# Chriz122/ultralytics_pro

Measured on AMD Instinct MI355X. Metric: images/sec (whole job = n_gpus x per-GPU bs=32) YOLOv8n 640x640 (forward + Detect decode + NMS), higher is better.
Workload: dtype bf16

## Files before the change

### include/upa.h

```cpp
#ifndef UPA_H
#define UPA_H
#include <stddef.h>
#include <stdint.h>

#ifdef __cplusplus
extern "C" {
#endif

enum { UPA_F32 = 0, UPA_BF16 = 1, UPA_U8_BGR_HWC = 2  };
enum { UPA_ACT_NONE = 0, UPA_ACT_SILU = 1, UPA_ACT_RELU = 2 };
enum { UPA_OK = 0, UPA_EINVAL = -1, UPA_EUNSUPPORTED = -2, UPA_EWORKSPACE = -3, UPA_ELAUNCH = -4 };

typedef struct upa_opts {
  uint32_t size;
  int32_t conv_big;
  int32_t conv_big_bm;
  int32_t conv_ckt;
  int32_t no_ws, no_pipe, no_1x1, no_c16, no_upcat;
  int32_t pipe_all;
  int32_t pipe_min_tiles;
  int32_t pipe_wgs, c16_wgs;
  int32_t c1_mt, c1_waves, c1_wgs;
  int32_t pair;
  int32_t pair_tile64, pair_tile32;
  int32_t no_pair_cv2;
  int32_t c2f;
  int32_t c2f16_waves;
  int32_t c2f32_th;
  int32_t no_branch_tail;
  int32_t branch_tail_bm;
  int32_t stem_wgs, stemf_wgs, stemf_waves, stem_no_mfma;
  int32_t ablate_conv, ablate_pipe, ablate_c1, ablate_stem;
  int32_t c2f64_max_px;
  int32_t conv_ws3;
  int32_t no_group;
  int32_t no_c2f32_up;
  int32_t no_xcd;
  int32_t keys_only;
  int32_t conv_p8;
  int32_t c2f_stream;
  int32_t c2f_stream_rows;
  int32_t no_stack_first;
  int32_t no_epi_stats;
  int32_t nms_stages;
  int32_t nms_first_prefix;
  int32_t detect_stream;
  int32_t detect_stream_rows;
  int32_t no_sppf_front;
  int32_t no_c2f16_down;
} upa_opts;

int upa_version(void);
const char* upa_last_error(void);
size_t upa_opts_size(void);

size_t upa_conv_packed_weight_bytes(int cout, int cin, int k, int dtype);
int upa_pack_conv_weight(const float* w_oihw, int cout, int cin, int k, int dtype, void* out);
int upa_conv2d_bias_act(const void* x, int n, int h, int w, int cin, int ldx,
                        const void* w_packed, const float* bias ,
                        void* y, int cout, int ldy,
                        const void* residual , int ldr,
                        int k, int stride, int pad, int act, int dtype, const upa_opts* opts, void* stream);
typedef struct upa_conv_problem {
  const void* x; int32_t n, h, w, cin, ldx;
  const void* w_packed; const float* bias;
  void* y; int32_t cout, ldy;
  const void* residual; int32_t ldr;
} upa_conv_problem;
int upa_conv2d_bias_act_group(const upa_conv_problem* probs, int count, int k, int stride, int pad, int act, int dtype,
                              const upa_opts* opts, void* stream);

int upa_conv2d_pool2(const void* x, int n, int h, int w, int cin, int ldx, const void* w_packed, const float* bias, void* y, int cout,
                     int ldy, int k, int stride, int pad, int act, int dtype, const upa_opts* opts, void* stream);
int upa_conv2d_stem_nchw_pool2(const void* x_nchw, int x_dtype, int n, int cin, int h, int w, const float* w_oihw, const float* bias,
                               void* y, int cout, int ldy, int k, int stride, int pad, int act, int dtype, const upa_opts* opts,
                               void* stream);

int upa_conv_variant(int n, int h, int w, int cin, int cout, int k, int stride, int pad, int dtype, const upa_opts* opts);

int upa_bottleneck_pair(const void* x, int n, int h, int w, int c, int ldx, const void* w1_packed, const float* b1,
                        const void* w2_packed, const float* b2, void* y, int ldy, int residual, int act, int dtype,
                        const upa_opts* opts, void* stream);
int upa_bottleneck_pair_e(const void* x, int n, int h, int w, int c, int cmid, int ldx, const void* w1_packed, const float* b1,
                          const void* w2_packed, const float* b2, void* y, int ldy, int residual, int act, int dtype,
                          const upa_opts* opts, void* stream);


size_t upa_stem_packed_weight_bytes(int cout, int cin, int k);
int upa_pack_stem_weight(const float* w_oihw, int cout, int cin, int k, float* out );
int upa_conv2d_stem_nchw(const void* x_nchw, int x_dtype, int n, int cin, int h, int w,
                         const float* w_oihw, const float* bias, void* y, int cout, int ldy,
                         int k, int stride, int pad, int act, int dtype, const upa_opts* opts, void* stream);

int upa_stem_conv_fused(const void* x, int n, int h, int w, const float* w0, const float* b0, const void* w1,
                        const float* b1, void* y, int ldy, const upa_opts* opts, void* stream);
int upa_stem_conv_fused_k(const void* x, int n, int h, int w, int k0, const float* w0, const float* b0, const void* w1,
                          const float* b1, void* y, int ldy, const upa_opts* opts, void* stream);
int upa_stem_conv_fused_c(const void* x, int n, int h, int w, int k0, int c0, const float* w0, const float* b0, const void* w1,
                          const float* b1, void* y, int ldy, const upa_opts* opts, void* stream);
int upa_stem_conv_fused_s(const void* x, int n, int h, int w, int k0, int s0, int c0, const float* w0, const float* b0,
                          const void* w1, const float* b1, void* y, int ldy, const upa_opts* opts, void* stream);

int upa_maxpool2d(const void* x, int n, int h, int w, int c, int ldx, void* y, int oh, int ow, int ldy,
                  int k, int stride, int pad, int pad_br, int dtype, void* stream);
int upa_sppf_pool3(const void* x, int n, int h, int w, int c, int ldx, void* y1, void* y2, void* y3, int ldy,
                   int dtype, void* stream);
int upa_sppf_front(const void* x, int n, int h, int w, int c1, int ldx, const void* w_packed, const float* bias, void* y, int c_, int ldy, int dtype,
                   const upa_opts* opts, void* stream);
int upa_upsample2x(const void* x, int n, int h, int w, int c, int ldx, void* y, int ldy, int dtype, void* stream);
int upa_copy_view(const void* x, int n, int h, int w, int c, int ldx, void* y, int ldy, int dtype, void* stream);
int upa_copy_to_host(const void* src_dev, void* dst_pinned, size_t bytes, void* stream);
int upa_results_to_host(const void* rows_dev, const int* counts_dev, int batch, int max_rows, int row_bytes,
                        void* rows_pinned, int* counts_pinned, void* stream);
int upa_add_view(const void* a, int lda, const void* b, int ldb, void* y, int ldy, int n, int h, int w, int c,
                 int dtype, void* stream);
int upa_nchw_to_nhwc(const float* x, int n, int c, int h, int w, void* y, int ldy, int dtype, void* stream);
int upa_nhwc_to_nchw(const void* x, int n, int h, int w, int c, int ldx, float* y, int dtype, void* stream);
int upa_letterbox_u8(const void* src, int n, int h0, int w0, long src_image_stride, int src_row_stride, void* dst, int H, int W,
                     int new_h, int new_w, int top, int left, int pad_value, void* stream);


int upa_detect_decode(const void* box, int ldb, const void* cls, int ldc, int n, int h, int w, int reg_max, int nc,
                      float stride_px, float* y, int a_total, int a0, int dtype, void* stream);
int upa_detect_tail(const void* x, int n, int h, int w, int cin, int ldx, const void* w_packed, const float* bias, int cout,
                    int kind, int nc, float stride_px, float* y, int a_total, int a0, void* raw, int ldraw,
                    unsigned long long* best_keys, int dtype, const upa_opts* opts, void* stream);

int upa_conv1x1_upcat(const void* x, int n, int h, int w, int cin, int ldx, const void* up, int up_c, int up_ld,
                      const void* w_packed, const float* bias, void* y, int cout, int ldy, int act, int dtype,
                      const upa_opts* opts, void* stream);

int upa_bottleneck_pair_cv2(const void* x, const void* y0, int n, int h, int w, int ldx, const void* w1_packed, const float* b1,
                            const void* w2_packed, const float* b2, int residual, const void* wc_std, const void* wc_b,
                            const float* bc, void* out, int ldout, int act, int dtype, const upa_opts* opts, void* stream);

int upa_c2f_fused(const void* x, int n, int h, int w, int c1, int ldx, int c, int nb, int shortcut, const void* w1,
                  const float* b1, const void* const* wm, const float* const* bm, const void* w2, const float* b2, void* y,
                  int c2, int ldy, int act, int dtype, const upa_opts* opts, void* stream);

int upa_c2f16_down_fused(const void* x, int n, int h, int w, int ldx, const void* w1, const float* b1, const void* const* wm,
                         const float* const* bm, const void* w2, const float* b2, const void* wd, const float* bd, void* y, int ldy,
                         int dtype, const upa_opts* opts, void* stream);

int upa_c2f64_fused(const void* x, int n, int h, int w, int c1, int ldx, const void* up, int up_c, int up_ld, int nb, int shortcut,
                    const void* w1, const float* b1, const void* const* wm, const float* const* bm, const void* w2,
                    const float* b2, void* y, int c2, int ldy, int act, int dtype, const upa_opts* opts, void* stream);
int upa_c2f32_up_fused(const void* x, int n, int h, int w, int c1, int ldx, const void* up, int up_c, int up_ld, int nb, int shortcut,
                       const void* w1, const float* b1, const void* const* wm, const float* const* bm, const void* w2, const float* b2,
                       void* y, int c2, int ldy, int act, int dtype, const upa_opts* opts, void* stream);

size_t upa_tail_packed_weight_bytes(int cout, int cin);
int upa_pack_tail_weight(const float* w, int cout, int cin, void* out);
int upa_detect_branch_tail(const void* x, int n, int h, int w, int c, int ldx, const void* w3_packed, const float* b3,
                           const void* wt_packed, const float* bt, int kind, int nc, float stride_px, float* y, int a_total,
                           int a0, unsigned long long* best_keys, int dtype, const upa_opts* opts, void* stream);
typedef struct upa_branch_level {
  const void* x; int32_t n, h, w, c, ldx;
  const void* w3_packed; const float* b3;
  const void* wt_packed; const float* bt;
  float stride_px; int32_t a0;
} upa_branch_level;
// ... 168 lines not shown
```

### ultralytics_pro_amd/_lib.py

```python

from __future__ import annotations

import ctypes as C
import os
from pathlib import Path

import torch

UPA_F32, UPA_BF16, UPA_U8_BGR_HWC = 0, 1, 2
UPA_EUNSUPPORTED = -2
ACT_NONE, ACT_SILU, ACT_RELU = 0, 1, 2

_PKG = Path(__file__).resolve().parent
LIB_PATH = Path(os.environ.get("UPA_HIP_LIB", _PKG / "libupa_hip.so"))

_vp, _i, _f, _sz = C.c_void_p, C.c_int, C.c_float, C.c_size_t


class Opts(C.Structure):

    _fields_ = [("size", C.c_uint32), ("conv_big", _i), ("conv_big_bm", _i), ("conv_ckt", _i),
                ("no_ws", _i), ("no_pipe", _i), ("no_1x1", _i), ("no_c16", _i), ("no_upcat", _i),
                ("pipe_all", _i), ("pipe_min_tiles", _i), ("pipe_wgs", _i), ("c16_wgs", _i),
                ("c1_mt", _i), ("c1_waves", _i), ("c1_wgs", _i),
                ("pair", _i), ("pair_tile64", _i), ("pair_tile32", _i), ("no_pair_cv2", _i),
                ("c2f", _i), ("c2f16_waves", _i), ("c2f32_th", _i),
                ("no_branch_tail", _i), ("branch_tail_bm", _i),
                ("stem_wgs", _i), ("stemf_wgs", _i), ("stemf_waves", _i), ("stem_no_mfma", _i),
                ("ablate_conv", _i), ("ablate_pipe", _i), ("ablate_c1", _i), ("ablate_stem", _i), ("c2f64_max_px", _i), ("conv_ws3", _i), ("no_group", _i), ("no_c2f32_up", _i), ("no_xcd", _i), ("keys_only", _i), ("conv_p8", _i), ("c2f_stream", _i), ("c2f_stream_rows", _i), ("no_stack_first", _i), ("no_epi_stats", _i), ("nms_stages", _i), ("nms_first_prefix", _i), ("detect_stream", _i), ("detect_stream_rows", _i), ("no_sppf_front", _i), ("no_c2f16_down", _i)]

    def __init__(self, **kw):
        super().__init__()
        self.size = C.sizeof(Opts)
        for k, v in kw.items():
            if k in dict(self._fields_):
                setattr(self, k, int(v))
            else:
                raise AttributeError(f"upa_opts has no field '{k}'")

    def replace(self, **kw) -> "Opts":
        o = Opts()
        C.memmove(C.byref(o), C.byref(self), C.sizeof(Opts))
        for k, v in kw.items():
            setattr(o, k, int(v))
        return o

    _ENV = {"UPA_CONV_BIG": ("conv_big", lambda v: {0: 1, 1: 0, 2: 2}[int(v)]), "UPA_CONV_BIG_BM": ("conv_big_bm", int), "UPA_CONV_WS3": ("conv_ws3", int),
            "UPA_CONV_CKT": ("conv_ckt", int), "UPA_CONV_NO_WS": ("no_ws", lambda v: 1), "UPA_CONV_NO_PIPE": ("no_pipe", lambda v: 1),
            "UPA_CONV_NO_1X1": ("no_1x1", lambda v: 1), "UPA_CONV_NO_C16": ("no_c16", lambda v: 1), "UPA_NO_UPCAT": ("no_upcat", lambda v: 1),
            "UPA_PIPE_ALL": ("pipe_all", lambda v: 1), "UPA_PIPE_MIN_TILES": ("pipe_min_tiles", int), "UPA_PIPE_WGS": ("pipe_wgs", int),
            "UPA_C16_WGS": ("c16_wgs", int), "UPA_C1_MT": ("c1_mt", int), "UPA_C1_WAVES": ("c1_waves", int), "UPA_C1_WGS": ("c1_wgs", int),
            "UPA_NO_PAIR": ("pair", lambda v: {0: 2, 1: 1, 2: 0, 3: 3}[int(v)]), "UPA_PAIR_T64": ("pair_tile64", int),
            "UPA_PAIR_T32": ("pair_tile32", int), "UPA_NO_PAIR_CV2": ("no_pair_cv2", int), "UPA_NO_C2F": ("c2f", int),
            "UPA_C2F16_WAVES": ("c2f16_waves", int), "UPA_C2F32_TH": ("c2f32_th", int), "UPA_NO_BRANCH_TAIL": ("no_branch_tail", int),
            "UPA_BRANCH_TAIL_BM": ("branch_tail_bm", int), "UPA_STEM_WGS": ("stem_wgs", int), "UPA_STEMF_WGS": ("stemf_wgs", int),
            "UPA_STEMF_WAVES": ("stemf_waves", int), "UPA_STEM_NO_MFMA": ("stem_no_mfma", lambda v: 1),
            "UPA_CONV_ABLATE": ("ablate_conv", int), "UPA_PIPE_ABLATE": ("ablate_pipe", int), "UPA_C1_ABLATE": ("ablate_c1", int),
            "UPA_STEM_ABLATE": ("ablate_stem", int)}

    @classmethod
    def from_env(cls, env=None) -> "Opts":
        env = os.environ if env is None else env
        o = cls()
        for name, (field, conv) in cls._ENV.items():
            if name in env:
                setattr(o, field, conv(env[name]))
        return o


class BranchLevel(C.Structure):
    _fields_ = [("x", C.c_void_p), ("n", _i), ("h", _i), ("w", _i), ("c", _i), ("ldx", _i), ("w3_packed", C.c_void_p), ("b3", C.c_void_p),
                ("wt_packed", C.c_void_p), ("bt", C.c_void_p), ("stride_px", C.c_float), ("a0", _i)]


class DetectBranch(C.Structure):
    _fields_ = [("c", _i), ("reserved", _i), ("w1", C.c_void_p), ("b1", C.c_void_p), ("w2", C.c_void_p), ("b2", C.c_void_p),
                ("wt", C.c_void_p), ("bt", C.c_void_p)]


class ConvProblem(C.Structure):
    _fields_ = [("x", C.c_void_p), ("n", _i), ("h", _i), ("w", _i), ("cin", _i), ("ldx", _i), ("w_packed", C.c_void_p), ("bias", C.c_void_p),
                ("y", C.c_void_p), ("cout", _i), ("ldy", _i), ("residual", C.c_void_p), ("ldr", _i)]


_op = C.POINTER(Opts)

PROTOTYPES = {
    "upa_version": (_i, []),
    "upa_last_error": (C.c_char_p, []),
    "upa_opts_size": (_sz, []),
    "upa_conv_packed_weight_bytes": (_sz, [_i, _i, _i, _i]),
    "upa_pack_conv_weight": (_i, [_vp, _i, _i, _i, _i, _vp]),
    "upa_conv2d_bias_act": (_i, [_vp, _i, _i, _i, _i, _i, _vp, _vp, _vp, _i, _i, _vp, _i, _i, _i, _i, _i, _i, _op, _vp]),
    "upa_conv_variant": (_i, [_i, _i, _i, _i, _i, _i, _i, _i, _i, _op]),
    "upa_bottleneck_pair": (_i, [_vp, _i, _i, _i, _i, _i, _vp, _vp, _vp, _vp, _vp, _i, _i, _i, _i, _op, _vp]),
    "upa_bottleneck_pair_e": (_i, [_vp, _i, _i, _i, _i, _i, _i, _vp, _vp, _vp, _vp, _vp, _i, _i, _i, _i, _op, _vp]),
    "upa_stem_packed_weight_bytes": (_sz, [_i, _i, _i]),
    "upa_pack_stem_weight": (_i, [_vp, _i, _i, _i, _vp]),
    "upa_conv2d_stem_nchw": (_i, [_vp, _i, _i, _i, _i, _i, _vp, _vp, _vp, _i, _i, _i, _i, _i, _i, _i, _op, _vp]),
    "upa_conv2d_stem_nchw_pool2": (_i, [_vp, _i, _i, _i, _i, _i, _vp, _vp, _vp, _i, _i, _i, _i, _i, _i, _i, _op, _vp]),
    "upa_conv2d_pool2": (_i, [_vp, _i, _i, _i, _i, _i, _vp, _vp, _vp, _i, _i, _i, _i, _i, _i, _i, _op, _vp]),
    "upa_stem_conv_fused": (_i, [_vp, _i, _i, _i, _vp, _vp, _vp, _vp, _vp, _i, _op, _vp]),
    "upa_stem_conv_fused_k": (_i, [_vp, _i, _i, _i, _i, _vp, _vp, _vp, _vp, _vp, _i, _op, _vp]),
    "upa_stem_conv_fused_c": (_i, [_vp, _i, _i, _i, _i, _i, _vp, _vp, _vp, _vp, _vp, _i, _op, _vp]),
    "upa_stem_conv_fused_s": (_i, [_vp, _i, _i, _i, _i, _i, _i, _vp, _vp, _vp, _vp, _vp, _i, _op, _vp]),
    "upa_maxpool2d": (_i, [_vp, _i, _i, _i, _i, _i, _vp, _i, _i, _i, _i, _i, _i, _i, _i, _vp]),
    "upa_sppf_pool3": (_i, [_vp, _i, _i, _i, _i, _i, _vp, _vp, _vp, _i, _i, _vp]),
    "upa_upsample2x": (_i, [_vp, _i, _i, _i, _i, _i, _vp, _i, _i, _vp]),
    "upa_copy_view": (_i, [_vp, _i, _i, _i, _i, _i, _vp, _i, _i, _vp]),
    "upa_copy_to_host": (_i, [_vp, _vp, _sz, _vp]),
    "upa_results_to_host": (_i, [_vp, _vp, _i, _i, _i, _vp, _vp, _vp]),
    "upa_add_view": (_i, [_vp, _i, _vp, _i, _vp, _i, _i, _i, _i, _i, _i, _vp]),
    "upa_nchw_to_nhwc": (_i, [_vp, _i, _i, _i, _i, _vp, _i, _i, _vp]),
    "upa_nhwc_to_nchw": (_i, [_vp, _i, _i, _i, _i, _i, _vp, _i, _vp]),
    "upa_letterbox_u8": (_i, [_vp, _i, _i, _i, C.c_long, _i, _vp, _i, _i, _i, _i, _i, _i, _i, _vp]),
    "upa_detect_decode": (_i, [_vp, _i, _vp, _i, _i, _i, _i, _i, _i, _f, _vp, _i, _i, _i, _vp]),
    "upa_detect_branch_tail_group": (_i, [_vp, _i, _i, _i, _vp, _i, _vp, _i, _op, _vp]),
    "upa_detect_head_tails": (_i, [_vp, _vp, _i, _i, _vp, _i, _vp, _i, _op, _vp]),
    "upa_conv2d_bias_act_group": (_i, [_vp, _i, _i, _i, _i, _i, _i, _op, _vp]),
    "upa_detect_level_stream": (_i, [_vp, _i, _i, _i, _i, _i, _vp, _vp, _i, _f, _vp, _i, _i, _vp, _i, _op, _vp]),
    "upa_detect_tail": (_i, [_vp, _i, _i, _i, _i, _i, _vp, _vp, _i, _i, _i, _f, _vp, _i, _i, _vp, _i, _vp, _i, _op, _vp]),
    "upa_conv1x1_upcat": (_i, [_vp, _i, _i, _i, _i, _i, _vp, _i, _i, _vp, _vp, _vp, _i, _i, _i, _i, _op, _vp]),
    "upa_bottleneck_pair_cv2": (_i, [_vp, _vp, _i, _i, _i, _i, _vp, _vp, _vp, _vp, _i, _vp, _vp, _vp, _vp, _i, _i, _i, _op, _vp]),
    "upa_sppf_front": (_i, [_vp, _i, _i, _i, _i, _i, _vp, _vp, _vp, _i, _i, _i, _op, _vp]),
    "upa_c2f16_down_fused": (_i, [_vp, _i, _i, _i, _i, _vp, _vp, _vp, _vp, _vp, _vp, _vp, _vp, _vp, _i, _i, _op, _vp]),
    "upa_c2f_fused": (_i, [_vp, _i, _i, _i, _i, _i, _i, _i, _i, _vp, _vp, _vp, _vp, _vp, _vp, _vp, _i, _i, _i, _i, _op, _vp]),
    "upa_c2f64_fused": (_i, [_vp, _i, _i, _i, _i, _i, _vp, _i, _i, _i, _i, _vp, _vp, _vp, _vp, _vp, _vp, _vp, _i, _i, _i, _i, _op, _vp]),
    "upa_c2f32_up_fused": (_i, [_vp, _i, _i, _i, _i, _i, _vp, _i, _i, _i, _i, _vp, _vp, _vp, _vp, _vp, _vp, _vp, _i, _i, _i, _i, _op, _vp]),
    "upa_tail_packed_weight_bytes": (_sz, [_i, _i]),
    "upa_pack_tail_weight": (_i, [_vp, _i, _i, _vp]),
    "upa_detect_branch_tail": (_i, [_vp, _i, _i, _i, _i, _i, _vp, _vp, _vp, _vp, _i, _i, _f, _vp, _i, _i, _vp, _i, _op, _vp]),
    "upa_nms_batched_hot": (_i, [_vp, _i, _i, _i, _f, _f, _i, _i, _vp, _i, _i, _f, _vp, _vp, _vp, _vp, _sz, _vp, _vp]),
    "upa_nms_workspace_bytes": (_sz, [_i, _i, _i, _i, _i]),
    "upa_nms_batched": (_i, [_vp, _i, _i, _i, _f, _f, _i, _i, _vp, _i, _i, _f, _vp, _vp, _vp, _vp, _sz, _vp]),
    "upa_nms_batched_opts": (_i, [_vp, _i, _i, _i, _f, _f, _i, _i, _vp, _i, _i, _f, _vp, _vp, _vp, _vp, _sz, _vp, _vp]),
    "upa_mhsa": (_i, [_vp, _vp, _vp, _i, _i, _i, _i, _i, _f, _vp, _i, _vp, _i, _i, _vp]),
    "upa_dwconv2d": (_i, [_vp, _i, _i, _i, _i, _i, _vp, _vp, _vp, _i, _i, _i, _i, _i, _i, _vp]),
    "upa_psa_attention": (_i, [_vp, _i, _i, _i, _i, _i, _i, _i, _f, _vp, _vp, _vp, _i, _i, _vp]),
    "upa_linear": (_i, [_vp, C.c_long, _i, _i, _vp, _vp, _vp, _i, _i, _vp, _i, _i, _vp]),
    "upa_linear_bf16": (_i, [_vp, C.c_long, _i, _i, _vp, _vp, _vp, _i, _i, _vp, _i, _i, _vp]),
    "upa_linear_mixed": (_i, [_vp, _i, C.c_long, _i, _i, _vp, _vp, _vp, _i, _i, _i, _vp, _i, _i, _vp]),
    "upa_layer_norm": (_i, [_vp, _vp, _i, _i, _vp, _vp, _f, _vp, _vp]),
    "upa_rows_add": (_i, [_vp, _vp, _vp, C.c_long, _i, _vp]),
    "upa_rows_scale": (_i, [_vp, _vp, _vp, C.c_long, _i, _vp]),
    "upa_rows_gather": (_i, [_vp, _vp, _vp, C.c_long, _i, _vp]),
    "upa_topk_tokens": (_i, [_vp, _i, _i, _vp, _i, _i, _vp, _vp, _vp]),
    "upa_box_refine": (_i, [_vp, _vp, _vp, C.c_long, _vp]),
    "upa_box_add_anchors": (_i, [_vp, _vp, _vp, _vp, C.c_long, _vp]),
    "upa_sigmoid": (_i, [_vp, _vp, C.c_long, _vp]),
    "upa_rtdetr_output": (_i, [_vp, _vp, _vp, C.c_long, _i, _vp]),
    "upa_rtdetr_postprocess": (_i, [_vp, _i, _i, _i, _f, _vp, _i, _vp, _f, _f, _vp, _vp, _vp]),
    "upa_msdeform_attn": (_i, [_vp, _vp, _i, _i, _i, _i, _vp, _vp, _vp, _i, _i, _vp, _vp]),
    "upa_msdeform_attn_strided": (_i, [_vp, _i, _i, _vp, _i, _i, _i, _i, _vp, _vp, _vp, _i, _i, _vp, _vp]),
    "upa_box_iou": (_i, [_vp, _i, _vp, _i, _f, _vp, _vp]),
    "upa_match_predictions": (_i, [_vp, _vp, _i, _i, _vp, _vp, _i, _vp, _i, _vp, _vp]),
    "upa_scale_boxes": (_i, [_vp, C.c_long, _i, _f, _f, _f, _i, _f, _f, _vp]),
    "upa_pack_conv_weight_dev": (_i, [_vp, _i, _i, _i, _i, _i, _vp, _vp]),
    "upa_channel_reduce_workspace_bytes": (_sz, [_i]),
    "upa_bn_stats": (_i, [_vp, C.c_long, _i, _i, _vp, _i, _vp]),
    "upa_bn_finalize": (_i, [_vp, C.c_long, _i, _f, _vp, _vp, _vp, _vp, _vp]),
    "upa_conv2d_bn_act_fwd": (_i, [_vp, _i, _i, _i, _i, _i, _vp, _vp, _i, _i, _i, _i, _i, _f, _vp, _vp, _vp, _vp, _vp, _vp, _f, _i, _vp, _i, _vp, _i,
                                    _vp, _i, _vp, _vp]),
    "upa_conv2d_bn_stats": (_i, [_vp, _i, _i, _i, _i, _i, _vp, _vp, _i, _i, _i, _i, _i, _f, _vp, _vp, _vp, _vp, _vp, _i, _vp, _vp]),
    "upa_bn_act_fwd": (_i, [_vp, C.c_long, _i, _i, _vp, _vp, _vp, _vp, _f, _i, _vp, _i, _vp, _i, _i, _vp]),
    "upa_bn_act_bwd": (_i, [_vp, _vp, C.c_long, _i, _i, _i, _vp, _vp, _vp, _vp, _f, _i, _vp, _i, _vp, _vp, _i, _vp, _i, _vp]),
    "upa_conv_bn_act_bwd": (_i, [_vp, _i, _i, _i, _i, _i, _vp, _vp, _i, _i, _i, _vp, _vp, _vp, _vp, _f, _i, _vp, _i, _vp, _vp, _vp, _vp, _vp, _sz,
                                  _vp, _vp, _vp, _i, _i, _i, _i, _i, _vp, _vp]),
    "upa_conv2d_dgrad_s2": (_i, [_vp, _i, _i, _i, _i, _i, _vp, _vp, _i, _i, _i, _i, _i, _i, _vp, _vp]),
    "upa_channel_sum": (_i, [_vp, C.c_long, _i, _i, _vp, _i, _vp, _i, _vp]),
    "upa_conv2d_wgrad_workspace_bytes": (_sz, [_i, _i, _i]),
    "upa_conv2d_wgrad": (_i, [_vp, _i, _i, _i, _i, _i, _vp, _i, _i, _vp, _i, _i, _i, _i, _i, _vp, _sz, _vp]),
    "upa_dilate2x": (_i, [_vp, _i, _i, _i, _i, _i, _vp, _i, _i, _i, _i, _vp]),
    "upa_dgrad_s2_phase_weights": (_i, [_vp, _i, _i, _vp, _vp]),
    "upa_interleave2x": (_i, [_vp, _vp, _vp, _vp, _i, _i, _i, _i, _i, _vp, _i, _i, _i, _i, _i, _vp]),
    "upa_upsample2x_bwd": (_i, [_vp, _i, _i, _i, _i, _i, _vp, _i, _i, _i, _vp]),
    "upa_maxpool2d_bwd_workspace_bytes": (_sz, [_i, _i, _i, _i, _i, _i, _i]),
    "upa_maxpool2d_bwd": (_i, [_vp, _vp, _i, _i, _i, _i, _i, _i, _i, _i, _i, _vp, _i, _i, _i, _vp, _sz, _vp]),
# ... 74 lines not shown
```

### ultralytics_pro_amd/csrc/conv.hip

```cpp
#include <stdlib.h>

#include <type_traits>

#include "common.h"
#include "conv_pipe.h"

struct ConvParams {
  const char* x;
  char* y;
  const char* res;
  const char* w;
  const float* bias;
  int N, H, W, Cin, ldx;
  int OH, OW, Cout, ldy, ldr;
  int KS, stride, pad;
  int TH, TW, tilesX, tilesY;
  int KTT;
  int CKT;
  int NTn;
  int act;
  int IH, IW, PS;
  unsigned magicIW;
  int tw_shift;
  int stageRows;
// ... 718 lines not shown

ConvPath conv_path(const ConvShape& s, const upa_opts* opts, ConvEntry entry, ConvPath from = ConvPath::WS3) {
  if (from <= ConvPath::WS3 && upa_conv_ws3_eligible(s, opts)) return ConvPath::WS3;
  if (from <= ConvPath::P8 && entry == ConvEntry::PLAIN && upa_conv_p8_eligible(s, opts)) return ConvPath::P8;
  if (from <= ConvPath::BIG && upa_conv_big_eligible(s, opts)) return ConvPath::BIG;
  if (from <= ConvPath::PIPE && upa_conv_pipe_eligible(s, opts)) return ConvPath::PIPE;
  if (from <= ConvPath::C1X1 && upa_conv1x1_eligible(s, opts)) return ConvPath::C1X1;
  return ConvPath::GENERIC;
}

BigParams big_params(const ConvShape& s, const void* x, const void* w_packed, const float* bias, void* y, const void* residual) {
  BigParams q;
  memset(&q, 0, sizeof(q));
  q.x = (const char*)x; q.y = (char*)y; q.res = (const char*)residual; q.w = (const char*)w_packed; q.bias = bias;
  q.N = s.n; q.H = s.h; q.W = s.w; q.Cin = s.cin; q.ldx = s.ldx; q.Cout = s.cout; q.ldy = s.ldy; q.ldr = s.ldr;
  q.OH = (s.h + 2 * s.pad - s.k) / s.stride + 1;
  q.OW = (s.w + 2 * s.pad - s.k) / s.stride + 1;
  q.KS = s.k; q.stride = s.stride; q.pad = s.pad; q.act = s.act;
  return q;
}

PipeParams pipe_params(const ConvShape& s, const void* x, const void* w_packed, const float* bias, void* y, const void* residual) {
  PipeParams q;
  memset(&q, 0, sizeof(q));
  q.x = (const char*)x; q.y = (char*)y; q.res = (const char*)residual; q.w = (const char*)w_packed; q.bias = bias;
  q.N = s.n; q.H = s.h; q.W = s.w; q.Cin = s.cin; q.ldx = s.ldx; q.Cout = s.cout; q.ldy = s.ldy; q.ldr = s.ldr; q.act = s.act;
  return q;
}

C1Params c1_params(const ConvShape& s, const void* x, const void* w_packed, const float* bias, void* y) {
  C1Params q;
  memset(&q, 0, sizeof(q));
  q.x = (const char*)x; q.y = (char*)y; q.w = (const char*)w_packed; q.bias = bias;
  q.Cin = s.cin; q.ldx = s.ldx; q.Cout = s.cout; q.ldy = s.ldy; q.act = s.act;
  return q;
}

int conv_check(const ConvShape& s) {
  UPA_CHECK_ARG(s.n > 0 && s.h > 0 && s.w > 0 && s.cin > 0 && s.cout > 0, "conv2d: bad shape");
  UPA_CHECK_ARG(s.k >= 1 && s.k <= 7 && s.stride >= 1 && s.stride <= 2 && s.pad >= 0 && s.pad < s.k, "conv2d: unsupported k/s/p");
  UPA_CHECK_ARG(s.dtype == UPA_F32 || s.dtype == UPA_BF16, "conv2d: bad dtype");
  const int E = 16 / upa_elem_size(s.dtype);
  UPA_CHECK_ARG(s.cin % E == 0 && s.ldx % E == 0, "conv2d: cin/ldx must be multiples of %d elements", E);
  UPA_CHECK_ARG(s.cout % E == 0 && s.ldy % E == 0 && s.ldr % E == 0,
                "conv2d: cout/ldy/ldr must be multiples of %d elements (16-byte row stores)", E);
  return UPA_OK;
}

int conv_generic(const ConvShape& s, const void* x, const void* w_packed, const float* bias, void* y, const void* residual,
                 const upa_opts* opts, void* stream, int query_only, int* variant) {
  ConvParams p;
  memset(&p, 0, sizeof(p));
  p.x = (const char*)x; p.y = (char*)y; p.res = (const char*)residual; p.w = (const char*)w_packed; p.bias = bias;
  p.N = s.n; p.H = s.h; p.W = s.w; p.Cin = s.cin; p.ldx = s.ldx;
  p.OH = (s.h + 2 * s.pad - s.k) / s.stride + 1;
  p.OW = (s.w + 2 * s.pad - s.k) / s.stride + 1;
  p.Cout = s.cout; p.ldy = s.ldy; p.ldr = s.ldr;
  p.KS = s.k; p.stride = s.stride; p.pad = s.pad; p.act = s.act;
  p.opts = opts;
#ifdef UPA_ABLATE
  p.ablate = UPA_OPT(opts, ablate_conv);
#endif
  const int ktch = 64 / upa_elem_size(s.dtype);
  p.KTT = cdiv(s.cin, ktch);
  p.NTn = cdiv(s.cout, 16);
  int ckt = (p.KTT % 4 == 0) ? 4 : ((p.KTT % 2 == 0) ? 2 : 1);
  if ((s.stride == 2 || p.NTn == 5 || p.NTn == 3) && ckt > 2) ckt = 2;
  if (s.k > 3 && ckt > 1) ckt = 1;
  if (const int v = UPA_OPT(opts, conv_ckt); (v == 1 || v == 2 || v == 4) && p.KTT % v == 0 && v <= ckt) ckt = v;
  p.CKT = ckt;
  hipStream_t st = (hipStream_t)stream;
  const int rc = s.dtype == UPA_BF16 ? dispatch_conv<bf16_t>(p, st, query_only, variant) : dispatch_conv<float>(p, st, query_only, variant);
  if (rc == UPA_EUNSUPPORTED) upa_set_error("conv2d: tile does not fit LDS (k=%d s=%d cin=%d)", s.k, s.stride, s.cin);
  return rc;
}

int conv_run(const ConvShape& s, const void* x, const void* w_packed, const float* bias, void* y, const void* residual,
             const upa_opts* opts, void* stream, int query_only, int* variant) {
  for (ConvPath path = conv_path(s, opts, ConvEntry::PLAIN);; path = conv_path(s, opts, ConvEntry::PLAIN, ConvPath((int)path + 1))) {
    int rc = UPA_EUNSUPPORTED;
    switch (path) {
      case ConvPath::WS3: rc = upa_conv_ws3_launch(big_params(s, x, w_packed, bias, y, residual), query_only, variant, stream, opts); break;
      case ConvPath::P8: rc = upa_conv_p8_launch(big_params(s, x, w_packed, bias, y, residual), query_only, variant, stream, opts); break;
      case ConvPath::BIG: rc = upa_conv_big_launch(big_params(s, x, w_packed, bias, y, residual), query_only, variant, stream, opts); break;
      case ConvPath::PIPE:
        return upa_conv_pipe_launch(pipe_params(s, x, w_packed, bias, y, residual), query_only, variant, stream, opts);
      case ConvPath::C1X1:
        return upa_conv1x1_launch(c1_params(s, x, w_packed, bias, y), s.n * s.h * s.w, query_only, variant, stream, opts);
      case ConvPath::GENERIC: return conv_generic(s, x, w_packed, bias, y, residual, opts, stream, query_only, variant);
    }
    if (rc != UPA_EUNSUPPORTED) return rc;
  }
}

}

extern "C" int upa_conv_variant(int n, int h, int w, int cin, int cout, int k, int stride, int pad, int dtype,
                                const upa_opts* opts) {
  const int E = 16 / upa_elem_size(dtype);
  const ConvShape s{n, h, w, cin, (cin + E - 1) / E * E, cout, cout, 0, k, stride, pad, UPA_ACT_NONE, dtype};
  if (const int rc = conv_check(s); rc != UPA_OK) return rc;
  int variant = 0;
  const int rc = conv_run(s, nullptr, nullptr, nullptr, nullptr, nullptr, opts, nullptr, 1, &variant);
  return rc == UPA_OK ? variant : rc;
}

extern "C" int upa_conv2d_bias_act(const void* x, int n, int h, int w, int cin, int ldx, const void* w_packed,
                                   const float* bias, void* y, int cout, int ldy, const void* residual, int ldr, int k,
                                   int stride, int pad, int act, int dtype, const upa_opts* opts, void* stream) {
  UPA_CHECK_ARG(x && w_packed && y, "conv2d: null pointer");
  UPA_CHECK_ARG(!residual || ldr > 0, "conv2d: residual without a pixel stride");
  const ConvShape s{n, h, w, cin, ldx, cout, ldy, residual ? ldr : 0, k, stride, pad, act, dtype};
  if (const int rc = conv_check(s); rc != UPA_OK) return rc;
  UPA_CHECK_ARG(((uintptr_t)x % 16 == 0) && ((uintptr_t)y % 16 == 0) && (!residual || (uintptr_t)residual % 16 == 0),
                "conv2d: misaligned view");
  return conv_run(s, x, w_packed, bias, y, residual, opts, stream, 0, nullptr);
}

int upa_bn_finalize_rows(const float* rows, int nrows, int ld, long npix, int c, float momentum, float* mean, float* var,
                         float* running_mean, float* running_var, void* stream);
extern "C" size_t upa_channel_reduce_workspace_bytes(int c);
extern "C" int upa_bn_stats(const void* z, long npix, int c, int ldz, double* ws, int dtype, void* stream);
extern "C" int upa_bn_finalize(const double* ws, long npix, int c, float momentum, float* mean, float* var, float* running_mean,
                               float* running_var, void* stream);
extern "C" int upa_conv2d_bn_stats(const void* x, int n, int h, int w, int cin, int ldx, const void* w_packed, void* z, int cout, int ldz,
                                   int k, int stride, int pad, float momentum, float* mean, float* var, float* running_mean,
                                   float* running_var, double* ws, int dtype, const upa_opts* opts, void* stream) {
  UPA_CHECK_ARG(x && w_packed && z && mean && var && ws, "conv2d_bn_stats: null pointer");
  UPA_CHECK_ARG(n > 0 && h > 0 && w > 0 && cin > 0 && cout > 0 && k >= 1 && stride >= 1, "conv2d_bn_stats: bad shape");
  const int oh = (h + 2 * pad - k) / stride + 1, ow = (w + 2 * pad - k) / stride + 1;
  const long npix = (long)n * oh * ow;
  const int mode = UPA_OPT(opts, no_epi_stats);
  if (!mode && dtype == UPA_BF16 && cout % 16 == 0 && ((uintptr_t)x % 16) == 0 && ((uintptr_t)z % 16) == 0) {
    float* rows = reinterpret_cast<float*>(ws);
    const long max_rows = (long)(upa_channel_reduce_workspace_bytes(cout) / ((size_t)2 * cout * sizeof(float)));
    const ConvShape s{n, h, w, cin, ldx, cout, ldz, 0, k, stride, pad, UPA_ACT_NONE, dtype};
    int nrows = 0, rc = UPA_EUNSUPPORTED;
    switch (conv_path(s, opts, ConvEntry::STATS)) {
      case ConvPath::WS3: {
        BigParams q = big_params(s, x, w_packed, nullptr, z, nullptr);
        q.stats = rows;
        rc = upa_conv_ws3_launch_stats(q, &nrows, max_rows, stream, opts);
        break;
      }
      case ConvPath::BIG: {
        BigParams q = big_params(s, x, w_packed, nullptr, z, nullptr);
        q.stats = rows;
        rc = upa_conv_big_launch_stats(q, &nrows, max_rows, stream, opts);
        break;
      }
      case ConvPath::C1X1: {
        C1Params q = c1_params(s, x, w_packed, nullptr, z);
        q.stats = rows;
        rc = upa_conv1x1_launch_stats(q, n * h * w, &nrows, max_rows, stream, opts);
        break;
      }
      default: break;
    }
    if (rc == UPA_OK) return upa_bn_finalize_rows(rows, nrows, cout, npix, cout, momentum, mean, var, running_mean, running_var, stream);
    if (rc != UPA_EUNSUPPORTED) return rc;
  }
  if (const int rc = upa_conv2d_bias_act(x, n, h, w, cin, ldx, w_packed, nullptr, z, cout, ldz, nullptr, 0, k, stride, pad, UPA_ACT_NONE,
                                         dtype, opts, stream); rc != UPA_OK)
    return rc;
  if (const int rc = upa_bn_stats(z, npix, cout, ldz, ws, dtype, stream); rc != UPA_OK) return rc;
  return upa_bn_finalize(ws, npix, cout, momentum, mean, var, running_mean, running_var, stream);
}

extern "C" int upa_conv2d_dgrad_s2(const void* dz, int n, int oh, int ow, int cout, int lddz, const void* phase_w_packed, void* dx, int h,
                                   int w, int cin, int lddx, int accumulate, int dtype, const upa_opts* opts, void* stream) {
  UPA_CHECK_ARG(dz && phase_w_packed && dx, "conv2d_dgrad_s2: null pointer");
  const ConvShape s{n, oh, ow, cout, lddz, 4 * cin, 4 * cin, 0, 2, 1, 1, UPA_ACT_NONE, dtype};
  if (dtype != UPA_BF16 || cin % 8 != 0 || lddx % 8 != 0 || lddz % 8 != 0 || ((uintptr_t)dz % 16) != 0 || ((uintptr_t)dx % 16) != 0 ||
      conv_path(s, opts, ConvEntry::PLAIN) != ConvPath::BIG)
    return UPA_EUNSUPPORTED;
  BigParams q = big_params(s, dz, phase_w_packed, nullptr, dx, accumulate ? dx : nullptr);
  q.ldy = lddx; q.ldr = lddx;
  q.il_h = h; q.il_w = w; q.il_c = cin;
  return upa_conv_big_launch_interleave(q, stream, opts);
}

extern "C" int upa_bn_act_fwd(const void* z, long npix, int c, int ldz, const float* mean, const float* var, const float* gamma,
                              const float* beta, float eps, int act, void* y, int ldy, const void* residual, int ldr, int dtype,
                              void* stream);
extern "C" int upa_conv2d_bn_act_fwd(const void* x, int n, int h, int w, int cin, int ldx, const void* w_packed, void* z, int cout, int ldz,
                                     int k, int stride, int pad, float momentum, float* mean, float* var, float* running_mean,
                                     float* running_var, const float* gamma, const float* beta, float eps, int act, void* y, int ldy,
// ... 62 lines not shown
```

### ultralytics_pro_amd/csrc/conv_pipe.h

```cpp
#pragma once
struct ConvShape {
  int n, h, w, cin, ldx, cout, ldy, ldr, k, stride, pad, act, dtype;
};
struct PipeParams {
  const char* x;
  char* y;
  const char* res;
  const char* w;
  const float* bias;
  int N, H, W, Cin, ldx, Cout, ldy, ldr;
  int KTT, NTn, nt0;
  int tilesX, tilesY, numTiles;
  int act;
  int pool;
#ifdef UPA_ABLATE
  int ablate;
#endif
};
bool upa_conv_pipe_eligible(const ConvShape& s, const upa_opts* opts);
int upa_conv_pipe_launch(PipeParams p, int query_only, int* variant, void* stream, const upa_opts* opts);

#include "detect_epi.h"
struct C1Params {
  const char* x;
  char* y;
  const char* w;
  const float* bias;
  int P;
  int Cin, ldx, Cout, ldy;
  int KTT, NTn, groups;
  int act;
#ifdef UPA_ABLATE
  int ablate;
#endif
  int epi;
  DetectEpi de;
  float* stats;
  int stats_ld;
  const char* up;
  int upKT, up_ld, upH, upW;
  unsigned upMagicW, upMagicH;
};
bool upa_conv1x1_eligible(const ConvShape& s, const upa_opts* opts);
int upa_conv1x1_launch(C1Params p, int n_pixels, int query_only, int* variant, void* stream, const upa_opts* opts);
int upa_conv1x1_launch_stats(C1Params p, int n_pixels, int* rows, long max_rows, void* stream, const upa_opts* opts);

struct BigParams {
  const char* x;
  char* y;
  const char* res;
  const char* w;
  const float* bias;
  int N, H, W, Cin, ldx, OH, OW, Cout, ldy, ldr;
  int KS, stride, pad;
  int TH, TW, tilesX, tilesY, IH, IW;
  int IWp;
  int HALF;
  int KTT, NTn;
  int act;
  unsigned magicTW, magicIW;
  int no_xcd;
  const char* tw;
  const float* tb;
  DetectEpi de;
  float* stats;
  int stats_ld;
  int il_h, il_w, il_c;
};
bool upa_conv_big_eligible(const ConvShape& s, const upa_opts* opts);
int upa_conv_big_launch(BigParams p, int query_only, int* variant, void* stream, const upa_opts* opts);
int upa_conv_big_launch_stats(BigParams p, int* rows, long max_rows, void* stream, const upa_opts* opts);
int upa_conv_big_launch_interleave(BigParams p, void* stream, const upa_opts* opts);
int upa_conv_big_launch_group(const BigParams* probs, int count, int* consumed, void* stream, const upa_opts* opts);

bool upa_conv_big_pick_tile(BigParams& p, int bm, int ntb, size_t lds_cap);

bool upa_conv_p8_eligible(const ConvShape& s, const upa_opts* opts);
int upa_conv_p8_launch(BigParams p, int query_only, int* variant, void* stream, const upa_opts* opts);

bool upa_conv_ws3_eligible(const ConvShape& s, const upa_opts* opts);
int upa_conv_ws3_launch(BigParams p, int query_only, int* variant, void* stream, const upa_opts* opts);
int upa_conv_ws3_launch_stats(BigParams p, int* rows, long max_rows, void* stream, const upa_opts* opts);

struct PairParams {
  const char* x;
  char* y;
  const char* w1;
  const char* w2;
  const float* b1;
  const float* b2;
  int N, H, W, OH, OW, ldx, ldy;
  int TH, TW, tilesX, tilesY;
  int IWp, MWp;
  unsigned magicIW, magicMW, magicTW;
  const char* y0;
  const char* wc_std;
  const char* wc_b;
  const float* bc;
  char* out; int ldout;
};
```

Measured before the change: 61190.

## Add dedicated 1x1 conv kernel with resident input and weight ring

Adds a specialised kernel for stride-1, unpadded 1x1 convolutions that reach the general BIG conv path. Each block stages its whole pixel tile's input channels into LDS once and streams weight slabs through a 3-deep LDS ring with async DMA, running MFMA over all output-channel blocks. The epilogue fuses bias, activation and residual using permlane swaps for packed bf16 stores. The intent is to avoid the generic conv tiling overhead for pointwise convs. Unsupported shapes fall back to the old kernel. The risk is higher LDS use lowering occupancy, and a fallback that depends on how rc is initialised.

```diff
diff --git a/include/upa.h b/include/upa.h
--- a/include/upa.h
+++ b/include/upa.h
@@ -48,6 +48,7 @@
   int32_t detect_stream_rows;
   int32_t no_sppf_front;
   int32_t no_c2f16_down;
+  int32_t conv_k1;
 } upa_opts;
 
 int upa_version(void);
@@ -77,6 +78,7 @@
                                void* stream);
 
 int upa_conv_variant(int n, int h, int w, int cin, int cout, int k, int stride, int pad, int dtype, const upa_opts* opts);
+int upa_conv_k1_variant(int n, int h, int w, int cin, int cout, int dtype, const upa_opts* opts);
 
 int upa_bottleneck_pair(const void* x, int n, int h, int w, int c, int ldx, const void* w1_packed, const float* b1,
                         const void* w2_packed, const float* b2, void* y, int ldy, int residual, int act, int dtype,
diff --git a/ultralytics_pro_amd/_lib.py b/ultralytics_pro_amd/_lib.py
--- a/ultralytics_pro_amd/_lib.py
+++ b/ultralytics_pro_amd/_lib.py
@@ -27,7 +27,7 @@
                 ("c2f", _i), ("c2f16_waves", _i), ("c2f32_th", _i),
                 ("no_branch_tail", _i), ("branch_tail_bm", _i),
                 ("stem_wgs", _i), ("stemf_wgs", _i), ("stemf_waves", _i), ("stem_no_mfma", _i),
-                ("ablate_conv", _i), ("ablate_pipe", _i), ("ablate_c1", _i), ("ablate_stem", _i), ("c2f64_max_px", _i), ("conv_ws3", _i), ("no_group", _i), ("no_c2f32_up", _i), ("no_xcd", _i), ("keys_only", _i), ("conv_p8", _i), ("c2f_stream", _i), ("c2f_stream_rows", _i), ("no_stack_first", _i), ("no_epi_stats", _i), ("nms_stages", _i), ("nms_first_prefix", _i), ("detect_stream", _i), ("detect_stream_rows", _i), ("no_sppf_front", _i), ("no_c2f16_down", _i)]
+                ("ablate_conv", _i), ("ablate_pipe", _i), ("ablate_c1", _i), ("ablate_stem", _i), ("c2f64_max_px", _i), ("conv_ws3", _i), ("no_group", _i), ("no_c2f32_up", _i), ("no_xcd", _i), ("keys_only", _i), ("conv_p8", _i), ("c2f_stream", _i), ("c2f_stream_rows", _i), ("no_stack_first", _i), ("no_epi_stats", _i), ("nms_stages", _i), ("nms_first_prefix", _i), ("detect_stream", _i), ("detect_stream_rows", _i), ("no_sppf_front", _i), ("no_c2f16_down", _i), ("conv_k1", _i)]
 
     def __init__(self, **kw):
         super().__init__()
@@ -93,6 +93,7 @@
     "upa_pack_conv_weight": (_i, [_vp, _i, _i, _i, _i, _vp]),
     "upa_conv2d_bias_act": (_i, [_vp, _i, _i, _i, _i, _i, _vp, _vp, _vp, _i, _i, _vp, _i, _i, _i, _i, _i, _i, _op, _vp]),
     "upa_conv_variant": (_i, [_i, _i, _i, _i, _i, _i, _i, _i, _i, _op]),
+    "upa_conv_k1_variant": (_i, [_i, _i, _i, _i, _i, _i, _op]),
     "upa_bottleneck_pair": (_i, [_vp, _i, _i, _i, _i, _i, _vp, _vp, _vp, _vp, _vp, _i, _i, _i, _i, _op, _vp]),
     "upa_bottleneck_pair_e": (_i, [_vp, _i, _i, _i, _i, _i, _i, _vp, _vp, _vp, _vp, _vp, _i, _i, _i, _i, _op, _vp]),
     "upa_stem_packed_weight_bytes": (_sz, [_i, _i, _i]),
diff --git a/ultralytics_pro_amd/csrc/conv.hip b/ultralytics_pro_amd/csrc/conv.hip
--- a/ultralytics_pro_amd/csrc/conv.hip
+++ b/ultralytics_pro_amd/csrc/conv.hip
@@ -824,7 +824,12 @@
     switch (path) {
       case ConvPath::WS3: rc = upa_conv_ws3_launch(big_params(s, x, w_packed, bias, y, residual), query_only, variant, stream, opts); break;
       case ConvPath::P8: rc = upa_conv_p8_launch(big_params(s, x, w_packed, bias, y, residual), query_only, variant, stream, opts); break;
-      case ConvPath::BIG: rc = upa_conv_big_launch(big_params(s, x, w_packed, bias, y, residual), query_only, variant, stream, opts); break;
+      case ConvPath::BIG: {
+        const BigParams q = big_params(s, x, w_packed, bias, y, residual);
+        if (s.k == 1 && !query_only) rc = upa_conv_k1_launch(q, 0, nullptr, stream, opts);
+        if (rc == UPA_EUNSUPPORTED) rc = upa_conv_big_launch(q, query_only, variant, stream, opts);
+        break;
+      }
       case ConvPath::PIPE:
         return upa_conv_pipe_launch(pipe_params(s, x, w_packed, bias, y, residual), query_only, variant, stream, opts);
       case ConvPath::C1X1:
@@ -845,6 +850,16 @@
   int variant = 0;
   const int rc = conv_run(s, nullptr, nullptr, nullptr, nullptr, nullptr, opts, nullptr, 1, &variant);
   return rc == UPA_OK ? variant : rc;
+}
+
+extern "C" int upa_conv_k1_variant(int n, int h, int w, int cin, int cout, int dtype, const upa_opts* opts) {
+  const int E = 16 / upa_elem_size(dtype);
+  const ConvShape s{n, h, w, cin, (cin + E - 1) / E * E, cout, cout, 0, 1, 1, 0, UPA_ACT_NONE, dtype};
+  if (const int rc = conv_check(s); rc != UPA_OK) return rc;
+  if (conv_path(s, opts, ConvEntry::PLAIN) != ConvPath::BIG) return 0;
+  int variant = 0;
+  const int rc = upa_conv_k1_launch(big_params(s, nullptr, nullptr, nullptr, nullptr, nullptr), 1, &variant, nullptr, opts);
+  return rc == UPA_OK ? variant : (rc == UPA_EUNSUPPORTED ? 0 : rc);
 }
 
 extern "C" int upa_conv2d_bias_act(const void* x, int n, int h, int w, int cin, int ldx, const void* w_packed,
diff --git a/ultralytics_pro_amd/csrc/conv_k1.hip b/ultralytics_pro_amd/csrc/conv_k1.hip
--- /dev/null
+++ b/ultralytics_pro_amd/csrc/conv_k1.hip
@@ -0,0 +1,265 @@
+#include <type_traits>
+
+#include "common.h"
+#include "conv_pipe.h"
+UPA_STAMP_DEFINE(conv_k1)
+
+constexpr int K1_RING = 3;
+
+struct K1Params {
+  const char* x;
+  char* y;
+  const char* res;
+  const char* w;
+  const float* bias;
+  int P;
+  int Cin, ldx, Cout, ldy, ldr;
+  int KTT, NTn, nChunks, nCB;
+  int biasBytes;
+  int act;
+};
+
+__device__ __forceinline__ void k1_wait_vm(const int n) {
+  switch (n) {
+#define K1_W(v) case v: asm volatile("s_waitcnt vmcnt(" #v ")" ::: "memory"); break;
+    K1_W(1) K1_W(2) K1_W(3) K1_W(4) K1_W(5) K1_W(6) K1_W(7) K1_W(8) K1_W(9) K1_W(10) K1_W(11) K1_W(12)
+    K1_W(13) K1_W(14) K1_W(15) K1_W(16) K1_W(17) K1_W(18) K1_W(19) K1_W(20) K1_W(21) K1_W(22) K1_W(23)
+#undef K1_W
+    default: asm volatile("s_waitcnt vmcnt(0)" ::: "memory"); break;
+  }
+}
+template <int N>
+__device__ __forceinline__ void k1_wait_vm_imm() {
+  static_assert(N >= 0 && N < 64, "vmcnt is a 6-bit field");
+  asm volatile("s_waitcnt vmcnt(%0)" ::"n"(N) : "memory");
+}
+
+template <int WM, int WN, int MT, int NT>
+__global__ __launch_bounds__(WM * WN * 64, 4) void conv_k1_kernel(const K1Params p) {
+  constexpr int NW = WM * WN;
+  constexpr int BM = WM * MT * 16;
+  constexpr int NB = WN * NT;
+  constexpr int SLAB = 2 * NB * 1024;
+  constexpr int SI = 2 * NB / NW;
+  constexpr int XI = BM * 8 / (64 * NW);
+  constexpr int XCH = BM * 128;
+  static_assert(SI * NW == 2 * NB && XI * NW * 64 == BM * 8 && (NT % 2) == 0, "pieces divide evenly over the waves; n-tiles in pairs");
+  extern __shared__ __attribute__((aligned(16))) char smem[];
+  const int tid = threadIdx.x;
+  const int lane = tid & 63;
+  const int wave = __builtin_amdgcn_readfirstlane(tid >> 6);
+  const int r = lane & 15, g = lane >> 4;
+  const int wm = wave / WN, wn = wave % WN;
+  const int tile0 = (int)blockIdx.x * BM;
+
+  const float* bl = reinterpret_cast<const float*>(smem);
+  char* ring = smem + p.biasBytes;
+  char* xs = ring + K1_RING * SLAB;
+
+  UPA_STAMP_AT(0);
+  UPA_STAMP_HWID();
+  for (int i = wave; i * 1024 < p.biasBytes; i += NW) {
+    const int co = (i * 64 + lane) * 4;
+    const char* src = reinterpret_cast<const char*>(g_zero16);
+    if (p.bias && co + 4 <= p.Cout) src = reinterpret_cast<const char*>(p.bias + co);
+    lds_dma16(src, smem + i * 1024);
+  }
+  const char* xsrc[XI];
+  int xcg[XI];
+#pragma unroll
+  for (int i = 0; i < XI; ++i) {
+    const int idx = (i * NW + wave) * 64 + lane;
+    const int pix = idx >> 3;
+    const int cg = (idx & 7) ^ (pix & 7);
+    const int gp = tile0 + pix;
+    xcg[i] = gp < p.P ? cg * 8 : (1 << 20);
+    xsrc[i] = p.x + ((size_t)(gp < p.P ? gp : 0) * (size_t)p.ldx + cg * 8) * 2;
+  }
+  auto stage_x = [&](int c) __attribute__((always_inline)) {
+#pragma unroll
+    for (int i = 0; i < XI; ++i) {
+      const char* src = reinterpret_cast<const char*>(g_zero16);
+      if (c * 64 + xcg[i] < p.Cin) src = xsrc[i] + c * 128;
+      lds_dma16(src, xs + c * XCH + (i * NW + wave) * 1024);
+    }
+  };
+  auto stage_w = [&](int cb, int c, int slot) __attribute__((always_inline)) {
+#pragma unroll
+    for (int i = 0; i < SI; ++i) {
+      const int f = i * NW + wave;
+      const int kt = f / NB, j = f - kt * NB;
+      const int ktg = c * 2 + kt;
+      const int nt = cb * NB + j;
+      const char* src = reinterpret_cast<const char*>(g_zero16);
+      if (cb < p.nCB && ktg < p.KTT && nt < p.NTn) src = p.w + (((size_t)ktg * p.NTn + nt) * 64 + lane) * 16;
+      lds_dma16(src, ring + slot * SLAB + f * 1024);
+    }
+  };
+
+  int icb = 0, ic = 0, islot = 0;
+  auto issue_next_slab = [&]() __attribute__((always_inline)) {
+    stage_w(icb, ic, islot);
+    if (++ic == p.nChunks) { ic = 0; ++icb; }
+    if (++islot == K1_RING) islot = 0;
+  };
+#pragma unroll
+  for (int c = 0; c < K1_RING - 1; ++c) {
+    if (c < p.nChunks) stage_x(c);
+    issue_next_slab();
+  }
+  for (int c = K1_RING - 1; c < p.nChunks; ++c) stage_x(c);
+
+  int paddr[MT];
+#pragma unroll
+  for (int i = 0; i < MT; ++i) paddr[i] = ((wm * MT + i) * 16 + r) * 128;
+  const int pswz = r & 7;
+
+  f32x4 acc[MT][NT];
+  int s = 0, slot = 0;
+  for (int cb = 0; cb < p.nCB; ++cb) {
+#pragma unroll
+    for (int i = 0; i < MT; ++i)
+#pragma unroll
+      for (int j = 0; j < NT; ++j) acc[i][j] = f32x4{0.f, 0.f, 0.f, 0.f};
+    for (int c = 0; c < p.nChunks; ++c, ++s) {
+      if (s < K1_RING - 1) {
+        const int later = p.nChunks - 1 - s;
+        k1_wait_vm(SI * (K1_RING - 2) + XI * (later > 0 ? later : 0));
+      } else {
+        k1_wait_vm_imm<SI * (K1_RING - 2)>();
+      }
+      asm volatile("s_waitcnt lgkmcnt(0)\n\ts_barrier" ::: "memory");
+      if (cb == 0 && c == 0) UPA_STAMP_AT(1);
+      if (cb == 0 && (c == 1 || p.nChunks == 1)) UPA_STAMP_AT(2);
+      issue_next_slab();
+      const char* wb = ring + slot * SLAB + (wn * NT) * 1024 + lane * 16;
+      const char* xb = xs + c * XCH;
+#pragma unroll
+      for (int kt = 0; kt < 2; ++kt) {
+        u32x4 a[NT], b[MT];
+#pragma unroll
+        for (int j = 0; j < NT; ++j) a[j] = *reinterpret_cast<const u32x4*>(wb + (kt * NB + j) * 1024);
+#pragma unroll
+        for (int i = 0; i < MT; ++i) b[i] = *reinterpret_cast<const u32x4*>(xb + paddr[i] + (((kt * 4 + g) ^ pswz) << 4));
+#pragma unroll
+        for (int i = 0; i < MT; ++i)
+#pragma unroll
+          for (int j = 0; j < NT; ++j) acc[i][j] = mfma32(a[j], b[i], acc[i][j]);
+      }
+      if (++slot == K1_RING) slot = 0;
+    }
+    if (cb == 0) UPA_STAMP_AT(3);
+
+    const int cw = (cb * NB + wn * NT) * 16;
+    f32x4 biasv[NT];
+#pragma unroll
+    for (int j = 0; j < NT; ++j) {
+      const int co = cw + j * 16 + g * 4;
+      biasv[j] = co < p.Cout ? *reinterpret_cast<const f32x4*>(bl + co) : f32x4{0.f, 0.f, 0.f, 0.f};
+    }
+    auto epilogue = [&](auto act_tag) __attribute__((always_inline)) {
+      constexpr int ACT = decltype(act_tag)::value;
+#pragma unroll
+      for (int i = 0; i < MT; ++i) {
+        const int gp = tile0 + (wm * MT + i) * 16 + r;
+        const bool pok = gp < p.P;
+        const size_t pixoff = (size_t)gp;
+        char* yrow = p.y + (pixoff * p.ldy + cw) * 2;
+        const char* rrow = p.res ? p.res + (pixoff * p.ldr + cw) * 2 : nullptr;
+#pragma unroll
+        for (int j = 0; j + 1 < NT; j += 2) {
+          const int cb8 = 16 * (j + (g & 1)) + 8 * (g >> 1);
+          float v0[4], v1[4];
+#pragma unroll
+          for (int q = 0; q < 4; ++q) {
+            v0[q] = act_rcp<ACT>(acc[i][j][q] + biasv[j][q]);
+            v1[q] = act_rcp<ACT>(acc[i][j + 1][q] + biasv[j + 1][q]);
+          }
+          const bool ok = pok && cw + cb8 < p.Cout;
+          char* dst = yrow + cb8 * 2;
+          if (p.res) {
+            float x8[8];
+#pragma unroll
+            for (int q = 0; q < 4; ++q) {
+              auto sw = __builtin_amdgcn_permlane16_swap(__float_as_uint(v0[q]), __float_as_uint(v1[q]), false, false);
+              x8[q] = __uint_as_float(sw[0]);
+              x8[4 + q] = __uint_as_float(sw[1]);
+            }
+            if (ok) {
+              const u32x4 rv = *reinterpret_cast<const u32x4*>(rrow + cb8 * 2);
+#pragma unroll
+              for (int q = 0; q < 4; ++q) {
+                x8[2 * q] += __uint_as_float(rv[q] << 16);
+                x8[2 * q + 1] += __uint_as_float(rv[q] & 0xFFFF0000u);
+              }
+              *reinterpret_cast<u32x4*>(dst) = u32x4{pack_bf16x2(x8[0], x8[1]), pack_bf16x2(x8[2], x8[3]),
+                                                     pack_bf16x2(x8[4], x8[5]), pack_bf16x2(x8[6], x8[7])};
+            }
+          } else {
+            auto lo = __builtin_amdgcn_permlane16_swap(pack_bf16x2(v0[0], v0[1]), pack_bf16x2(v1[0], v1[1]), false, false);
+            auto hi = __builtin_amdgcn_permlane16_swap(pack_bf16x2(v0[2], v0[3]), pack_bf16x2(v1[2], v1[3]), false, false);
+            if (ok) *reinterpret_cast<u32x4*>(dst) = u32x4{lo[0], hi[0], lo[1], hi[1]};
+          }
+        }
+      }
+    };
+    if (p.act == UPA_ACT_SILU) epilogue(std::integral_constant<int, UPA_ACT_SILU>{});
+    else if (p.act == UPA_ACT_RELU) epilogue(std::integral_constant<int, UPA_ACT_RELU>{});
+    else epilogue(std::integral_constant<int, UPA_ACT_NONE>{});
+    if (cb == 0) UPA_STAMP_AT(4);
+  }
+  UPA_STAMP_AT(5);
+  asm volatile("s_waitcnt vmcnt(0)" ::: "memory");
+  UPA_STAMP_AT(6);
+}
+
+namespace {
+template <int WM, int WN, int MT, int NT>
+int k1_launch_inst(const K1Params& p, size_t lds, hipStream_t s) {
+  constexpr int BM = WM * MT * 16;
+  if (hipError_t e = upa_full_lds<conv_k1_kernel<WM, WN, MT, NT>>(); e != hipSuccess) {
+    upa_set_error("conv_k1: cannot raise LDS limit: %s", hipGetErrorString(e));
+    return UPA_ELAUNCH;
+  }
+  hipLaunchKernelGGL((conv_k1_kernel<WM, WN, MT, NT>), dim3((unsigned)cdiv(p.P, BM)), dim3(WM * WN * 64), lds, s, p);
+  UPA_LAUNCH_CHECK();
+  return UPA_OK;
+}
+size_t k1_lds_bytes(const K1Params& p, int bm, int nb) {
+  return (size_t)p.biasBytes + (size_t)K1_RING * (2 * nb * 1024) + (size_t)p.nChunks * bm * 128;
+}
+}
+
+int upa_conv_k1_launch(const BigParams& q, int query_only, int* variant, void* stream, const upa_opts* opts) {
+  const int mode = UPA_OPT(opts, conv_k1);
+  if (mode == 1) return UPA_EUNSUPPORTED;
+  const long px = (long)q.N * q.H * q.W;
+  if (q.KS != 1 || q.stride != 1 || q.pad != 0 || q.Cin > 512 || q.stats || q.tw || px + 128 >= (1L << 31) ||
+      q.Cin % 8 != 0 || q.ldx % 8 != 0 || q.Cout % 8 != 0 || q.ldy % 8 != 0 || q.ldr % 8 != 0 ||
+      (q.act != UPA_ACT_SILU && q.act != UPA_ACT_NONE && q.act != UPA_ACT_RELU))
+    return UPA_EUNSUPPORTED;
+  K1Params p;
+  memset(&p, 0, sizeof(p));
+  p.x = q.x; p.y = q.y; p.res = q.res; p.w = q.w; p.bias = q.bias;
+  p.P = (int)px; p.Cin = q.Cin; p.ldx = q.ldx; p.Cout = q.Cout; p.ldy = q.ldy; p.ldr = q.ldr; p.act = q.act;
+  p.KTT = cdiv(q.Cin, 32);
+  p.NTn = cdiv(q.Cout, 16);
+  p.nChunks = (p.KTT + 1) / 2;
+  p.biasBytes = cdiv(p.NTn * 64, 1024) * 1024;
+  const size_t half = 80 * 1024 - 512;
+  const int nb_wide = p.NTn > 4 ? 8 : 4;
+  int bm = 0, nb = 0;
+  const int cand[4][2] = {{128, nb_wide}, {128, 4}, {64, nb_wide}, {64, 4}};
+  for (int i = 0; i < 4 && !bm; ++i)
+    if (k1_lds_bytes(p, cand[i][0], cand[i][1]) <= half) { bm = cand[i][0]; nb = cand[i][1]; }
+  if (!bm) { bm = 64; nb = 4; }
+  if (mode >= 2 && mode <= 5) { bm = mode <= 3 ? 128 : 64; nb = (mode & 1) ? 4 : 8; }
+  const size_t lds = k1_lds_bytes(p, bm, nb);
+  if (lds > 160 * 1024 - 512) return UPA_EUNSUPPORTED;
+  p.nCB = cdiv(p.NTn, nb);
+  if (variant) *variant = (1 << 27) | (nb << 4) | (bm >> 6);
+  if (query_only) return UPA_OK;
+  hipStream_t s = (hipStream_t)stream;
+  if (bm == 128) return nb == 8 ? k1_launch_inst<4, 2, 2, 4>(p, lds, s) : k1_launch_inst<4, 2, 2, 2>(p, lds, s);
+  return nb == 8 ? k1_launch_inst<2, 2, 2, 4>(p, lds, s) : k1_launch_inst<2, 2, 2, 2>(p, lds, s);
+}
diff --git a/ultralytics_pro_amd/csrc/conv_pipe.h b/ultralytics_pro_amd/csrc/conv_pipe.h
--- a/ultralytics_pro_amd/csrc/conv_pipe.h
+++ b/ultralytics_pro_amd/csrc/conv_pipe.h
@@ -73,6 +73,8 @@
 int upa_conv_big_launch_interleave(BigParams p, void* stream, const upa_opts* opts);
 int upa_conv_big_launch_group(const BigParams* probs, int count, int* consumed, void* stream, const upa_opts* opts);
 
+int upa_conv_k1_launch(const BigParams& q, int query_only, int* variant, void* stream, const upa_opts* opts);
+
 bool upa_conv_big_pick_tile(BigParams& p, int bm, int ntb, size_t lds_cap);
 
 bool upa_conv_p8_eligible(const ConvShape& s, const upa_opts* opts);
```

Result: no change. 61370 (median of 6 runs) (+0.3%).
